# Franc-Z/CuClarabel

Measured on AMD Instinct MI355X. Metric: KKT factorize+solve/sec (fp64) per IPM iter, 100k-var SOCP, higher is better.
Workload: dtype f64

## Files before the change

cuclarabel_amd/csrc/factor_kernels.hip:

```cpp
#include "kernels.hpp"
#include "knobs.hpp"
#include <utility>

namespace hipkkt {

__device__ inline double rl_f64(double v, int lane)
{
    const int lo = __builtin_amdgcn_readlane(__double2loint(v), lane);
    const int hi = __builtin_amdgcn_readlane(__double2hiint(v), lane);
    return __hiloint2double(hi, lo);
}
#define WAVE_FENCE() asm volatile("" ::: "memory")

__device__ __forceinline__ void lds_add(double* p, double v)
{
    __hip_atomic_fetch_add(p, v, __ATOMIC_RELAXED, __HIP_MEMORY_SCOPE_WORKGROUP);
}
#define OV_LD(p) __hip_atomic_load((p), __ATOMIC_RELAXED, __HIP_MEMORY_SCOPE_AGENT)
#define OV_ST(p, v) __hip_atomic_store((p), (v), __ATOMIC_RELAXED, __HIP_MEMORY_SCOPE_AGENT)
__device__ inline bool ov_wait_ge(const int* counter, int target, int* abort_word, long long t0, long long limit, int who = 0, int info = 0,
                                  int* seen_min = nullptr)
{
    for (;;) {
        const int seen = __hip_atomic_load(counter, __ATOMIC_RELAXED, __HIP_MEMORY_SCOPE_AGENT);
// ... 4 lines not shown
            return false;
        }
        __builtin_amdgcn_s_sleep(2);
    }
}
__device__ inline int lower_bound_dev(const int* __restrict__ arr, int n, int v)
{
    int lo = 0, hi = n;
    while (lo < hi) {
        const int mid = (lo + hi) >> 1;
        if (arr[mid] < v) lo = mid + 1; else hi = mid;
    }
    return lo;
}

__global__ __launch_bounds__(256) void k_front_wave(FactorArgs A, int begin, int count, int slice)
{
    extern __shared__ __attribute__((aligned(16))) double smem[];
    const int lane = threadIdx.x & 63, wv = threadIdx.x >> 6;
    const int item = blockIdx.x * 4 + wv;
    if (item >= count) return;
    const TreeDev& T = A.T;
    const FrontDesc fd = T.desc[begin + item];
    const int s = fd.s, c0 = fd.c0, nc = fd.nc, nb = fd.nb;
    const int f = nc + nb;
    double* __restrict__ F = A.fronts + fd.front_off;
    double* __restrict__ U = A.upd + fd.upd_off;
    double* P = smem + (size_t)wv * slice;
    double* Us = P + f * nc;

    const bool pulled_leaf = (fd.pad & 2) != 0;
    for (int i = lane; i < f * nc + (pulled_leaf ? 0 : nb * nb); i += 64) P[i] = 0.0;
    WAVE_FENCE();
    {
        const int64_t e0 = fd.kptr;
        const int ne = fd.nk;
        for (int e = lane; e < ne; e += 64) P[T.kdst[e0 + e]] = A.Kval[T.ksrc[e0 + e]];
    }
    WAVE_FENCE();
    if (A.eps) {
        const double eps = *A.eps;
        if (lane < nc) P[lane + lane * f] += eps * (double)T.psign[c0 + lane];
    }
// ... 64 lines not shown
        WAVE_FENCE();
    }
    for (int i = lane; i < f * nc; i += 64) {
        const int j = i / f, r = i - j * f;
        if (r >= j) F[i] = P[i];
    }
    if (lane < nb && !pulled_leaf) {
        const int a = lane;
        for (int b = 0; b <= a; ++b) {
            double acc = 0.0;
            for (int k = 0; k < nc; ++k) acc = fma(P[nc + a + k * f] * P[k + k * f], P[nc + b + k * f], acc);
            U[a + (int64_t)b * nb] = Us[a + b * nb] - acc;
        }
    }
}

constexpr int kTinySlice = 128;
__global__ __launch_bounds__(256) void k_front_tiny(FactorArgs A, int begin, int count)
{
    __shared__ __attribute__((aligned(16))) double smem_t[32 * kTinySlice];
    const int sub = threadIdx.x & 7, grp = threadIdx.x >> 3;
    const int item = blockIdx.x * 32 + grp;
    if (item >= count) return;
    const TreeDev& T = A.T;
    const FrontDesc fd = T.desc[begin + item];
    const int s = fd.s, c0 = fd.c0, nc = fd.nc, nb = fd.nb;
    const int f = nc + nb;
    double* __restrict__ F = A.fronts + fd.front_off;
    double* __restrict__ U = A.upd + fd.upd_off;
    double* P = smem_t + grp * kTinySlice;
    double* Us = P + f * nc;

    const bool pulled_leaf = (fd.pad & 2) != 0;
    for (int i = sub; i < f * nc + (pulled_leaf ? 0 : nb * nb); i += 8) P[i] = 0.0;
    WAVE_FENCE();
    {
        const int64_t e0 = fd.kptr;
        const int ne = fd.nk;
        for (int e = sub; e < ne; e += 8) P[T.kdst[e0 + e]] = A.Kval[T.ksrc[e0 + e]];
    }
    WAVE_FENCE();
    if (A.eps) {
        const double eps = *A.eps;
        if (sub < nc) P[sub + sub * f] += eps * (double)T.psign[c0 + sub];
    }
// ... 38 lines not shown
        WAVE_FENCE();
    }
    for (int i = sub; i < f * nc; i += 8) {
        const int j = i / f, r = i - j * f;
        if (r >= j) F[i] = P[i];
    }
    if (sub < nb && !pulled_leaf) {
        const int a = sub;
        for (int b = 0; b <= a; ++b) {
            double acc = 0.0;
            for (int k = 0; k < nc; ++k) acc = fma(P[nc + a + k * f] * P[k + k * f], P[nc + b + k * f], acc);
            U[a + (int64_t)b * nb] = Us[a + b * nb] - acc;
        }
    }
}

typedef double d4_t __attribute__((ext_vector_type(4)));

__device__ inline double fast_recip(double d)
{
    double r = __builtin_amdgcn_rcp(d);
    r = fma(fma(-d, r, 1.0), r, r);
    r = fma(fma(-d, r, 1.0), r, r);
    return r;
}
constexpr int NB = kPanelNB;
__device__ __forceinline__ int pcol(int j, int f) { return (j * (2 * f - 1 - j)) >> 1; }

__device__ inline int64_t uniform_i64(int64_t v)
{
// ... 101 lines not shown
{
    int lo = __double2loint(v), hi = __double2hiint(v);
    switch (k) {
        HIPKKT_BCAST16_CASE(0) HIPKKT_BCAST16_CASE(1) HIPKKT_BCAST16_CASE(2) HIPKKT_BCAST16_CASE(3)
        HIPKKT_BCAST16_CASE(4) HIPKKT_BCAST16_CASE(5) HIPKKT_BCAST16_CASE(6) HIPKKT_BCAST16_CASE(7)
        HIPKKT_BCAST16_CASE(8) HIPKKT_BCAST16_CASE(9) HIPKKT_BCAST16_CASE(10) HIPKKT_BCAST16_CASE(11)
        HIPKKT_BCAST16_CASE(12) HIPKKT_BCAST16_CASE(13) HIPKKT_BCAST16_CASE(14) HIPKKT_BCAST16_CASE(15)
    }
    return __hiloint2double(hi, lo);
}

template <int BS, bool SLICED, bool OV>
__global__ __launch_bounds__(BS) void k_panel(FactorArgs A, int begin)
{
    extern __shared__ __attribute__((aligned(16))) double smem[];
    const int tid = threadIdx.x, lane = tid & 63;
    const int wv = __builtin_amdgcn_readfirstlane(tid >> 6);
    constexpr int NW = BS / 64;
    constexpr int NWK = NW - NW / 4;
    const int widx = wv - 1 - (wv >> 2);
    const TreeDev& T = A.T;
    const FrontDesc fd = SLICED ? T.sdesc[begin + blockIdx.x] : T.desc[begin + blockIdx.x];
    const int s = fd.s, c0 = fd.c0, nc = fd.nc, nb = fd.nb;
    const int ff = nc + nb;
    const int nsl = SLICED ? (fd.pad & 0xffff) : 1, sl = SLICED ? (fd.pad >> 16) : 0;
    const int rsmax = (nb + nsl - 1) / nsl;
    const int r_lo = nc + sl * rsmax;
    const int rs = SLICED ? max(0, min(rsmax, ff - r_lo)) : nb;
    const int f = nc + rs;
    const bool first = !SLICED || sl == 0;
    double* __restrict__ F = A.fronts + fd.front_off;
    if (OV && tid == 0) __hip_atomic_fetch_add(A.ov_started + A.ov_slot, 1, __ATOMIC_RELAXED, __HIP_MEMORY_SCOPE_AGENT);

    double* sh_d_all = smem;
    double* sh_dinv_all = smem + 2 * NB;
    double* Lb_all = smem + 4 * NB;
    double* colb = smem + 4 * NB + 2 * NB * NB;
    double* sgn = colb + 4 * NB;
    int* lds_cnt = reinterpret_cast<int*>(sgn + kBdCols + NB);
    double* P = sgn + kBdCols + NB + 2;

    HIPKKT_STAMP(A, 0);
    const long long clk0 = A.stamps ? clock64() : 0;
    const int64_t dense_off_s = T.dense_off[s];
    int64_t it0 = 0, it1 = 0;
    int pt0 = 0, pt1 = 0;
    PullGroup pt_first{};
    ExtItem it_first{};
    {
        const int64_t* __restrict__ wc = T.wave_cut + (int64_t)(SLICED ? T.nsuper + begin + (int)blockIdx.x : s) * 17;
        constexpr int SPW = 16 / NW > 0 ? 16 / NW : 1;
        if (wv * SPW < 16) {
            it0 = wc[wv * SPW];
            it1 = wc[min(16, (wv + 1) * SPW)];
            if (it1 > it0) it_first = T.items[min(it0 + lane, it1 - 1)];
            if (!SLICED) {
                pt0 = T.pwave_cut[(int64_t)s * 17 + wv * SPW];
                pt1 = T.pwave_cut[(int64_t)s * 17 + min(16, (wv + 1) * SPW)];
                pt0 = __builtin_amdgcn_readfirstlane(pt0);
                pt1 = __builtin_amdgcn_readfirstlane(pt1);
                if (pt1 > pt0) pt_first = pull_fetch(T.pterms, pt0, pt1, lane);
            }
        }
    }
    for (int k = tid; k < nc; k += BS) sgn[k] = (double)T.psign[c0 + k];
    const int psize = f * nc - ((nc * (nc - 1)) >> 1);
    for (int i = tid; i < psize; i += BS) P[i] = 0.0;
    __syncthreads();
    HIPKKT_STAMP(A, 1);
    {
        const int64_t e0 = fd.kptr;
        const int ne = fd.nk;
        for (int base = 0; base < ne; base += 4 * BS) {
            int src[4], dst[4];
            double v[4];
#pragma unroll
            for (int q = 0; q < 4; ++q) {
                const int e = base + q * BS + tid;
                src[q] = e < ne ? T.ksrc[e0 + e] : -1;
                dst[q] = e < ne ? T.kdst[e0 + e] : -1;
            }
#pragma unroll
            for (int q = 0; q < 4; ++q) v[q] = src[q] >= 0 ? A.Kval[src[q]] : 0.0;
#pragma unroll
            for (int q = 0; q < 4; ++q) if (dst[q] >= 0) P[dst[q]] = v[q];
        }
    }
    __syncthreads();
    if (A.eps) {
        const double eps = *A.eps;
        for (int k = tid; k < nc; k += BS) P[k + pcol(k, f)] += eps * sgn[k];
    }
    __syncthreads();
    HIPKKT_STAMP(A, 2);
    if (OV) {
        volatile int& sh_ov_ok = reinterpret_cast<volatile int*>(lds_cnt)[2];
        if (tid == 0) sh_ov_ok = 1;
        __syncthreads();
        if (wv == 0) {
            const long long tw = wall_clock64();
            bool ok = true;
            for (int e = T.child_ptr[s] + lane; e < T.child_ptr[s + 1]; e += 64) {
                const int c = T.child_idx[e];
                const int need = A.ov_ntiles[c];
                if (need > 0) ok = ov_wait_ge(A.ov_done + c, need, A.flags + 2, tw, A.ov_limit, 1, c) && ok;
            }
            if (!ok) sh_ov_ok = 0;
        }
        __syncthreads();
// ... 10 lines not shown
#pragma unroll
                for (int q = 0; q < 8; ++q) {
                    const int idx = base + q * BS + tid;
                    const int j = idx / f, rl = idx - j * f;
                    const int r = (!SLICED || rl < nc) ? rl : r_lo + (rl - nc);
                    const bool ok = idx < total && rl >= j;
                    tg[q] = ok ? rl + pcol(j, f) : -1;
                    v[q] = ok ? (OV ? OV_LD(Uc + r + (int64_t)j * ff) : Uc[r + (int64_t)j * ff]) : 0.0;
                }
#pragma unroll
                for (int q = 0; q < 8; ++q) if (tg[q] >= 0) P[tg[q]] += v[q];
            }
            __syncthreads();
        }
    }
    if (A.stamps && blockIdx.x == 0 && tid == 0) {
        asm volatile("s_waitcnt vmcnt(0)" ::: "memory");
        A.stamps[A.stamp_row * 16 + 6] = wall_clock64();
    }
    if (!SLICED && pt1 > pt0) apply_pulled(T.pterms, A.fronts, P, pt0, pt1, lane, pt_first);
    if (it1 > it0) apply_items_panel<SLICED, OV>(T, A.upd, P, f, it0, it1, lane, nc, r_lo, rs, it_first,
                                             (A.stamps && blockIdx.x == 0 && wv == 0) ? A.stamps + A.stamp_row * 16 + 15 : nullptr);
    if (A.stamps && blockIdx.x == 0 && tid == 0) A.stamps[A.stamp_row * 16 + 7] = wall_clock64();
    HIPKKT_STAMP(A, 3);
    long long t_i = 0, t_ii = 0, t_iii = 0, t0 = 0;
    auto diag_block = [&](const int kb, const int w, const int par) {
        double* sh_d = sh_d_all + par * NB;
        double* sh_dinv = sh_dinv_all + par * NB;
        double* Tb = Lb_all + par * NB * NB;
        int lane_o = lane;
        const int i = lane & 15, g = lane >> 4;
        const double my_sg = (lane < w) ? sgn[kb + lane] : 1.0;
        int nreg = 0;
        bool bad = false;
        double a4[4], lout[4], t4[4];
#pragma unroll
        for (int q = 0; q < 4; ++q) {
            const int j = 4 * g + q;
            a4[q] = (i < w && j <= i) ? P[(kb + i) + pcol(kb + j, f)] : 0.0;
// ... 129 lines not shown
                WAVE_FENCE();
                for (int idx = widx * 64 + lane; idx < w * f; idx += NWK * 64) {
                    const int jj = idx / f, r = idx - jj * f, j = kb + jj;
                    if (!SLICED) {
                        if (r >= j) OV_ST(F + r + (int64_t)j * ff, P[r + pcol(j, f)]);
                    } else if (r >= nc) {
                        OV_ST(F + (r_lo + r - nc) + (int64_t)j * ff, P[r + pcol(j, f)]);
                    } else if (first && r >= j) {
                        OV_ST(F + r + (int64_t)j * ff, P[r + pcol(j, f)]);
                    }
                }
                asm volatile("s_waitcnt vmcnt(0)" ::: "memory");
                if (lane == 0) {
                    const int arrived = __hip_atomic_fetch_add(lds_cnt + 1, 1, __ATOMIC_RELAXED, __HIP_MEMORY_SCOPE_WORKGROUP) + 1;
                    if (arrived == NWK * epoch)
                        __hip_atomic_store(SLICED ? A.ov_sprog + begin + blockIdx.x : A.ov_prog + s, kb + w, __ATOMIC_RELAXED,
                                           __HIP_MEMORY_SCOPE_AGENT);
                }
            }
            if (Tc > 0) {
                while (__hip_atomic_load(lds_cnt, __ATOMIC_RELAXED, __HIP_MEMORY_SCOPE_WORKGROUP) < (NWK + 1) * epoch)
                    __builtin_amdgcn_s_sleep(1);
                WAVE_FENCE();
                const int ntr = (Tr + 15) >> 4, ntc = (Tc + 15) >> 4;
                for (int t = widx; t < ntr * ntc; t += NWK) {
                    const int tc = t / ntr, tr = t - tc * ntr;
                    if (tr < tc || (tr == 0 && tc == 0)) continue;
                    tile(tr, tc);
                }
            }
        }
        if (A.stamps) { long long t1 = wall_clock64(); t_iii += t1 - t0; }
    }
    __syncthreads();
    HIPKKT_STAMP(A, 4);
    if (!OV) for (int idx = tid; idx < f * nc; idx += BS) {
        const int j = idx / f, r = idx - j * f;
        if (!SLICED) {
            if (r >= j) F[idx] = P[r + pcol(j, f)];
        } else if (r >= nc) {
            F[(r_lo + r - nc) + (int64_t)j * ff] = P[r + pcol(j, f)];
        } else if (first && r >= j) {
            F[r + (int64_t)j * ff] = P[r + pcol(j, f)];
        }
    }
    __syncthreads();
    HIPKKT_STAMP(A, 5);
    if (A.stamps && blockIdx.x == 0 && tid == 0) {
        A.stamps[A.stamp_row * 16 + 8] = t_i;
        A.stamps[A.stamp_row * 16 + 9] = t_ii;
        A.stamps[A.stamp_row * 16 + 10] = t_iii;
        A.stamps[A.stamp_row * 16 + 11] = f;
        A.stamps[A.stamp_row * 16 + 12] = nc;
        A.stamps[A.stamp_row * 16 + 13] = T.child_ptr[s + 1] - T.child_ptr[s];
        A.stamps[A.stamp_row * 16 + 14] = clock64() - clk0;
    }
}

constexpr int TS = 64;
constexpr int KC = 16;

constexpr int LDA = TS + 16;

// ... 230 lines not shown
static void init_factor_lds()
{
    static PerDeviceOnce once;
    once.run([]() {
        hipError_t e = hipSuccess;
        auto set = [&](auto k) { if (e == hipSuccess) e = set_max_lds(k, 160 * 1024); };
        set(k_panel<256, false, false>);
        set(k_panel<512, false, false>);
        set(k_panel<1024, false, false>);
        set(k_panel<256, false, true>);
        set(k_panel<512, false, true>);
        set(k_panel<1024, false, true>);
        set(k_panel<1024, true, false>);
        set(k_panel<1024, true, true>);
        set(k_front_wave);
        return e;
    });
}

void launch_front_tiny(const FactorArgs& a, int begin, int count, hipStream_t st)
{
    if (count <= 0) return;
    hipLaunchKernelGGL(k_front_tiny, dim3((count + 31) / 32), dim3(256), 0, st, a, begin, count);
}
void launch_front_wave(const FactorArgs& a, int begin, int count, int slice_doubles, hipStream_t st)
{
    if (count <= 0) return;
    init_factor_lds();
    hipLaunchKernelGGL(k_front_wave, dim3((count + 3) / 4), dim3(256), (size_t)4 * slice_doubles * sizeof(double), st,
                       a, begin, count, slice_doubles);
}
void launch_panel(const FactorArgs& a, int begin, int count, int bs, size_t lds, hipStream_t st)
{
    if (count <= 0) return;
    init_factor_lds();
    if (a.ov) {
        if (bs == 1024) hipLaunchKernelGGL((k_panel<1024, false, true>), dim3(count), dim3(1024), lds, st, a, begin);
        else if (bs == 512) hipLaunchKernelGGL((k_panel<512, false, true>), dim3(count), dim3(512), lds, st, a, begin);
        else hipLaunchKernelGGL((k_panel<256, false, true>), dim3(count), dim3(256), lds, st, a, begin);
        return;
    }
    if (bs == 1024) hipLaunchKernelGGL((k_panel<1024, false, false>), dim3(count), dim3(1024), lds, st, a, begin);
    else if (bs == 512) hipLaunchKernelGGL((k_panel<512, false, false>), dim3(count), dim3(512), lds, st, a, begin);
    else hipLaunchKernelGGL((k_panel<256, false, false>), dim3(count), dim3(256), lds, st, a, begin);
}
void launch_panel_sliced(const FactorArgs& a, int begin, int count, size_t lds, hipStream_t st)
{
    if (count <= 0) return;
    init_factor_lds();
    if (a.ov) hipLaunchKernelGGL((k_panel<1024, true, true>), dim3(count), dim3(1024), lds, st, a, begin);
    else hipLaunchKernelGGL((k_panel<1024, true, false>), dim3(count), dim3(1024), lds, st, a, begin);
}
void launch_schur(const FactorArgs& a, const int2* tiles, int tile_begin, int ntiles, hipStream_t st, int ov_grid, int tile_nc)
{
    if (ntiles <= 0) return;
    const int pipe_tiles = knobs().schur_pipe_tiles;
    const int pipe_nc = knobs().schur_pipe_nc;
    if (a.ov) hipLaunchKernelGGL((k_schur<true, true>), dim3(std::max(1, std::min(ntiles, ov_grid))), dim3(256), 0, st, a, tiles, tile_begin, ntiles);
    else if (ntiles > pipe_tiles && tile_nc >= pipe_nc) hipLaunchKernelGGL((k_schur<false, true>), dim3(ntiles), dim3(256), 0, st, a, tiles, tile_begin, ntiles);
// ... 65 lines not shown
```

cuclarabel_amd/csrc/hipkkt.hip:

```cpp
#include "../../include/hipkkt.h"

#include <hip/hip_runtime.h>

#include <algorithm>
#include <cfloat>
#include <chrono>
#include <climits>
#include <cmath>
#include <cstdio>
#include <cstdlib>
#include <cstring>
#include <array>
#include <functional>
#include <map>
#include <memory>
#include <mutex>
#include <stdexcept>
#include <string>
#include <vector>

#include "kernels.hpp"
#include "kkt_assembly.hpp"
#include "symbolic.hpp"
#include "knobs.hpp"
// ... 100 lines not shown
            }
            if (knobs().verbose >= 2)
                for (size_t q = 0; q < sch.launches.size(); ++q) {
                    const Launch& L = sch.launches[q];
                    int fmin = 1 << 30, ncmin = 1 << 30;
                    double flops = 0;
                    for (int t = L.begin; t < L.begin + L.count; ++t) {
                        const int sn = sch.sched[(size_t)t], nc = S.sn_start[sn + 1] - S.sn_start[sn], f = front_size(sn);
                        fmin = std::min(fmin, f); ncmin = std::min(ncmin, nc);
                        flops += (double)nc * (f - nc) * (f - nc) + (double)nc * nc * (f - nc) + (double)nc * nc * nc / 3;
                    }
                    std::fprintf(stderr, "[hipkkt] launch %zu level %d: %d fronts (%s), f %d..%d, nc %d..%d, %d sliced into %d, %d tiles (%d columns deep on average), %.3f GF\n",
                                 q, L.level, L.count, L.small ? "one wave" : "block", fmin, L.fmax, ncmin, L.ncmax, L.nsliced, L.slice_count,
                                 L.ntiles, L.tile_nc, flops * 1e-9);
                }
            if (overlap_wanted())
                for (size_t q = sch.ov_first; q < sch.launches.size(); ++q)
                    std::fprintf(stderr, "[hipkkt] overlap admission: launch %zu: %d panel workgroups, %d tiles behind a gate, %d CUs\n", q,
                                 sch.ov_group_of[q] >= 0 ? sch.ov_groups[(size_t)sch.ov_group_of[q]].count : sch.launches[q].count - sch.launches[q].nsliced + sch.launches[q].slice_count,
                                 sch.launches[q].ntiles, dev.n_cus);
        }
    }

    void factor(const double* d_Kval, const double* d_eps)
    {
        const bool want_stamps = knobs().stamps;
        const bool no_graph = !knobs().graph;
        if (want_stamps || no_graph || n_factor_calls++ == 0) {
            enqueue_factor(d_Kval, d_eps, stream, nullptr, want_stamps);
            return;
// ... 329 lines not shown
                    if (g->sliced) launch_panel_sliced(a, L.slice_begin, g->count, g->lds, st);
                    else launch_panel(a, L.begin, g->count, 1024, g->lds, st);
                }
                if (q == sch.ov_first) {
                    HIP_CHECK(hipEventRecord(ev_ov_fork, st));
                    HIP_CHECK(hipStreamWaitEvent(ov_stream, ev_ov_fork, 0));
                } else if (L.ntiles > 0 && !no_gate) {
                    if (merged) launch_ov_gate(d_ov_started.p + g->first, g->count, flags.p + 2, ov_limit, ov_stream);
                    else launch_ov_gate(d_ov_started.p + q, L.count - L.nsliced + L.slice_count, flags.p + 2, ov_limit, ov_stream);
                }
                launch_schur(a, (const int2*)d_tiles.p, L.tile_begin, L.ntiles, ov_stream, L.ntiles);
                a.ov = 0;
                continue;
            }
            if (L.small) {
                launch_front_wave(a, L.begin, L.count - L.ntiny, L.slice, st);
                launch_front_tiny(a, L.begin + L.count - L.ntiny, L.ntiny, st);
            } else {
                a.nbk = L.nbk;
                launch_panel(a, L.begin, L.count - L.nsliced, L.bs_panel, L.lds_panel, st);
                launch_panel_sliced(a, L.slice_begin, L.slice_count, L.lds_sliced, st);
                if (L.tinv_count > 0 && side) {
                    HIP_CHECK(hipEventRecord(ev_fork, st));
                    HIP_CHECK(hipStreamWaitEvent(side, ev_fork, 0));
                    form_w(d_tinv_list.p + L.tinv_begin, L.tinv_count, L.tinv_ncmax, side, 0);
                    forked = true;
                }
                launch_schur(a, (const int2*)d_tiles.p, L.tile_begin, L.ntiles, st, 0, L.tile_nc);
            }
        }
        if (forked) {
            HIP_CHECK(hipEventRecord(ev_join, side));
            HIP_CHECK(hipStreamWaitEvent(st, ev_join, 0));
        } else if (eager_fork) {
            const int done = w_done;
// ... 4091 lines not shown
```

cuclarabel_amd/csrc/kernels.hpp:

```cpp
#pragma once
#include <hip/hip_runtime.h>
#include "launch_shapes.hpp"
#include <cstdint>
#include <mutex>
#include <stdexcept>
#include <string>

namespace hipkkt {

struct HipError : std::runtime_error { using std::runtime_error::runtime_error; };

class PerDeviceOnce {
    std::mutex mu_;
    uint64_t done_[4] = {0, 0, 0, 0};
public:
    template <class F>
    void run(F&& fn)
    {
        int dev = 0;
        if (hipGetDevice(&dev) != hipSuccess || dev < 0 || dev >= 256) throw HipError("hipGetDevice failed");
        std::lock_guard<std::mutex> lk(mu_);
        if (done_[dev >> 6] >> (dev & 63) & 1) return;
        const hipError_t e = fn();
        if (e != hipSuccess) {
// ... 86 lines not shown
    double* fronts;
    double* upd;
    double* Dinv;
    int* flags;
    int* ov_prog;
    int* ov_done;
    const int* ov_ntiles;
    int* ov_sprog;
    const int* ov_sbase;
    int* ov_started;
    int ov_slot;
    int ov;
    long long ov_limit;
    double dyn_eps, dyn_delta;
    int nbk;
    long long* stamps;
    int stamp_row;
};
#define HIPKKT_STAMP(A, k) do { if ((A).stamps && blockIdx.x == 0 && threadIdx.x == 0) \
        (A).stamps[(A).stamp_row * 16 + (k)] = wall_clock64(); } while (0)

struct SolveArgs {
    TreeDev T;
    const double* fronts;
    const double* tinv;
    const double* Dinv;
    const double* b;
    double* out;
    double* xp;
    double* uvec;
    long long* top_stamps;
    long long top_limit;
    int64_t ld_b, ld_out, ld_xp, ld_uvec;
    const int* tk_pos;
// ... 7 lines not shown
};

constexpr int kSolveChunk = 128;
int top_solve_capacity(size_t lds, bool tall);
int top_solve_capacity_nr(size_t lds_total, int nr);
void launch_top_solve(const SolveArgs& a, int begin, int count, int grid, size_t lds, int* flags, int nflag, int epoch,
                      hipStream_t st, bool tall, int nr = 1);
int top_solve_sliced_capacity(size_t lds, int nr = 1);
void launch_top_solve_sliced(const SolveArgs& a, int begin, int pos0, int task0, int task1, int grid, size_t lds, int* flags, int nflag,
                             int epoch, hipStream_t st, int nr = 1);
void launch_tinv(const TreeDev& T, const double* fronts, double* tinv, const int* list, int count, int ncmax,
                 hipStream_t st, int max_blocks = 0, int nsmall = 0);

void launch_front_wave(const FactorArgs& a, int begin, int count, int slice_doubles, hipStream_t st);
void launch_front_tiny(const FactorArgs& a, int begin, int count, hipStream_t st);
void launch_panel(const FactorArgs& a, int begin, int count, int bs, size_t lds, hipStream_t st);
void launch_panel_sliced(const FactorArgs& a, int begin, int count, size_t lds, hipStream_t st);
void launch_schur(const FactorArgs& a, const int2* tiles, int tile_begin, int ntiles, hipStream_t st, int ov_grid = 0, int tile_nc = 0);
void launch_ov_gate(const int* started, int target, int* abort_word, long long limit, hipStream_t st);
void launch_concurrency_probe(int* word2, hipStream_t first, hipStream_t second);
void launch_handover_litmus(int variant, double* payload, int* sig, int* ack, int pairs, int words, int rounds,
                            unsigned long long* mismatches, unsigned long long* timeouts, hipStream_t st);
void launch_fwd(const SolveArgs& a, const RecSeg& rs, int begin, int count, int bs, size_t lds, hipStream_t st, int nr = 1);
void launch_bwd(const SolveArgs& a, const RecSeg& rs, int begin, int count, int bs, size_t lds, hipStream_t st, int nr = 1);
void launch_fwd_small(const SolveArgs& a, const RecSeg& rs, int begin, int nwave, int ntiny, hipStream_t st, bool leaf = false, int nr = 1);
void launch_bwd_small(const SolveArgs& a, const RecSeg& rs, int begin, int nwave, int ntiny, hipStream_t st, int nr = 1);
void launch_fwd_level(const SolveArgs& a, const RecSeg& rs, int begin, int nblock, int nwave, int ntiny, int bs, size_t lds, hipStream_t st, int nr = 1);
void launch_bwd_level(const SolveArgs& a, const RecSeg& rs, int begin, int nblock, int nwave, int ntiny, int bs, size_t lds, hipStream_t st, int nr = 1);

void launch_permute_in(const double* B, int64_t ldb, double* Xp, int KP, const int* iperm, int N, int nrhs, hipStream_t st);
// ... 299 lines not shown
```

cuclarabel_amd/csrc/knobs.hpp:

```cpp
#pragma once
#include <cstdlib>

namespace hipkkt {

#define HIPKKT_KNOBS(KNOB, FLAG_SET, FLAG_ON)                                                                                         \
                                                                                                                 \
    KNOB(int, verbose, "HIPKKT_VERBOSE", 0)                  \
    FLAG_SET(stamps, "HIPKKT_STAMPS")                                    \
    KNOB(int, top_stamps, "HIPKKT_TOP_STAMPS", 0)            \
    KNOB(int, top_stamps_nr, "HIPKKT_TOP_STAMPS_NR", 1)                                       \
    FLAG_SET(dump_levels, "HIPKKT_DUMP_LEVELS")                                \
    FLAG_SET(dump_subtrees, "HIPKKT_DUMP_SUBTREES")                        \
                                                                                      \
    KNOB(double, nd_sep_ratio, "HIPKKT_ND_SEP_RATIO", 0.10)  \
    KNOB(int, nd_sep_min, "HIPKKT_ND_SEP_MIN", 5000)                                           \
    KNOB(long long, panel_cap, "HIPKKT_PANEL_CAP", -1)       \
    KNOB(int, panel_max_cols, "HIPKKT_PANEL_MAX_COLS", -1)                                                  \
    KNOB(int, panel_slice_below, "HIPKKT_PANEL_SLICE_BELOW", -1)  \
    FLAG_SET(postorder_layout, "HIPKKT_POSTORDER_LAYOUT")                       \
    FLAG_ON(upd_pingpong, "HIPKKT_UPD_PINGPONG")                                        \
    KNOB(int, bundle_kids, "HIPKKT_BUNDLE_KIDS", 200)        \
    KNOB(int, bundle_kids_panel, "HIPKKT_BUNDLE_KIDS_PANEL", 400)   \
    FLAG_ON(bundle_cost, "HIPKKT_BUNDLE_COST")               \
                                                                                                  \
// ... 14 lines not shown
    FLAG_SET(graph, "HIPKKT_GRAPH")                               \
    FLAG_SET(no_overlap, "HIPKKT_NO_OVERLAP")                                                         \
    KNOB(int, winv_tail, "HIPKKT_WINV_TAIL", 4)                \
    KNOB(int, winv_early, "HIPKKT_WINV_EARLY", 1)                                                   \
    KNOB(int, winv_blocks, "HIPKKT_WINV_BLOCKS", 0)                           \
    FLAG_ON(winv_split, "HIPKKT_WINV_SPLIT")                 \
    FLAG_ON(winv_run_forks, "HIPKKT_WINV_RUN_FORKS")                        \
    FLAG_ON(factor_overlap, "HIPKKT_FACTOR_OVERLAP")                 \
    FLAG_SET(ov_cu_mask, "HIPKKT_OV_CU_MASK")                                        \
    KNOB(long long, ov_test_limit, "HIPKKT_OV_TEST_LIMIT", 5000000)   \
    KNOB(int, ov_max_fronts, "HIPKKT_OV_MAX_FRONTS", 0)      \
    KNOB(int, ov_max_tiles, "HIPKKT_OV_MAX_TILES", 1600)     \
    KNOB(int, ov_merge, "HIPKKT_OV_MERGE", 100)                   \
    KNOB(int, ov_merge_wide, "HIPKKT_OV_MERGE_WIDE", 24)                     \
    KNOB(int, ov_merge_groups, "HIPKKT_OV_MERGE_GROUPS", 8)                                \
    KNOB(int, schur_pipe_tiles, "HIPKKT_SCHUR_PIPE_TILES", 1600)                     \
    KNOB(int, schur_pipe_nc, "HIPKKT_SCHUR_PIPE_NC", 64)            \
                                                                                                                      \
    FLAG_SET(no_top, "HIPKKT_NO_TOP")                                                            \
    KNOB(int, top_tall, "HIPKKT_TOP_TALL", -1)                                        \
    KNOB(int, top_cap, "HIPKKT_TOP_CAP", 1 << 30)                                        \
    KNOB(double, top_mult, "HIPKKT_TOP_MULT", 1.5)                            \
    KNOB(long long, top_test_limit, "HIPKKT_TOP_TEST_LIMIT", 5000000)  \
    FLAG_SET(no_level_merge, "HIPKKT_NO_LEVEL_MERGE")               \
    KNOB(int, solve_slice_kb, "HIPKKT_SOLVE_SLICE_KB", 80)                                  \
    KNOB(int, solve_slice_max, "HIPKKT_SOLVE_SLICE_MAX", 64)                                     \
    KNOB(long long, solve_slice_from, "HIPKKT_SOLVE_SLICE_FROM", -1)  \
    FLAG_ON(chain, "HIPKKT_CHAIN")                                                           \
    FLAG_ON(chain_top, "HIPKKT_CHAIN_TOP")                   \
    KNOB(int, chain_max, "HIPKKT_CHAIN_MAX", 640)                                             \
// ... 35 lines not shown
```

cuclarabel_amd/csrc/launch_shapes.hpp:

```cpp
#pragma once
#include <cstddef>
#include <cstdint>

namespace hipkkt {

constexpr size_t kLdsCap = 160 * 1024 - 512;

constexpr int kLongRow = 4096;
constexpr int kLongChunk = 2048;

constexpr int kSmallFrontMax = 64;
constexpr int kSmallSliceMax = 1536;

constexpr int kPanelNB = 16;
constexpr int kMaxNbk = 16;
constexpr int kBdCols = 128;
inline size_t panel_lds_bytes(int fmax, int panel_max)
{
    (void)fmax;
    return ((size_t)8 * kPanelNB + 2 * kPanelNB * kPanelNB + (kBdCols + kPanelNB) + 2 + (size_t)panel_max + 256) * sizeof(double);
}

inline size_t solve_lds_bytes(int fmax, int ncmax)
{
    const size_t fpad = (size_t)((fmax + 3) & ~3), ncpad = (size_t)((ncmax + 3) & ~3);
    const size_t nks = (size_t)((ncmax + 7) >> 3), nrs = (size_t)((fmax + 7) >> 3);
    const size_t fwd = fpad + nks * fpad, bwd = fpad + nrs * ncpad;
// ... 60 lines not shown
```

cuclarabel_amd/csrc/schedule.cpp:

```cpp
#include "schedule.hpp"

#include <algorithm>
#include <cstdio>
#include <stdexcept>
#include <unordered_map>

namespace hipkkt {

static bool front_is_tall(const Symbolic& S, int s)
{
    const int tall_rows = knobs().solve_tall_rows;
    const int f = front_size(S, s), nc = S.sn_start[s + 1] - S.sn_start[s];
    return solve_lds_bytes(f, nc) > kLdsCap || (tall_rows > 0 && f >= tall_rows);
}

static void form_launches(const Symbolic& S, const DeviceLimits& dev, int64_t panel_cap, int panel_max_slices, Schedule& sch)
{
    sch.tile_base.assign(S.nsuper, -1);
    auto ncols = [&](int s) { return S.sn_start[s + 1] - S.sn_start[s]; };
    auto is_small = [&](int s) {
        int f = front_size(S, s), nc = ncols(s), nb = f - nc;
        return f <= kSmallFrontMax && f * nc + nb * nb <= kSmallSliceMax;
    };
    int level_no = -1;
// ... 276 lines not shown
        const int wgs = chain_seg_wgs(L.small ? 0 : L.count, L.small ? L.count - L.ntiny : 0, L.small ? L.ntiny : 0);
        if (L.ntall > 0 || (!L.small && L.lds_solve > 150 * 1024) || wgs > chain_max) break;
        if (!L.small) sch.chain_lds = std::max(sch.chain_lds, L.lds_solve);
        --q;
    }
    sch.chain_from = sch.launches.size() - q >= 2 ? q : sch.launches.size();
    sch.nch.assign((size_t)std::max(S.nsuper, 1), 0);
    if (sch.chain_from < sch.launches.size()) {
        const int p0 = sch.launches[sch.chain_from].begin;
        for (int c = 0; c < S.nsuper; ++c)
            if (S.sn_parent[c] >= 0 && sch.spos[(size_t)c] >= p0) sch.nch[(size_t)S.sn_parent[c]]++;
    }
}


Schedule build_schedule(const Symbolic& S, const DeviceLimits& dev, int64_t panel_cap, int panel_max_slices)
{
    Schedule sch;
    form_launches(S, dev, panel_cap, panel_max_slices, sch);
    admit_overlap(dev, sch);
    pick_late(sch);
    pick_top(S, dev, sch);
    pick_chain(S, sch);
    sch.rec_bytes = layout_records(sch.launches, &sch.rec_refused_bytes);
    return sch;
}

int rec_classes(const Launch& L, RecClass out[2])
{
    int n = 0;
    if (L.small) {
        if (L.count - L.ntiny > 0) out[n++] = {L.begin, L.count - L.ntiny, 1};
        if (L.ntiny > 0) out[n++] = {L.begin + L.count - L.ntiny, L.ntiny, 2};
    } else if (L.count > 0) {
        out[n++] = {L.begin, L.count, 0};
// ... 474 lines not shown
```

cuclarabel_amd/csrc/schedule.hpp:

```cpp
#pragma once
#include <array>
#include <cstddef>
#include <cstdint>
#include <functional>
#include <string>
#include <vector>

#include "knobs.hpp"
#include "launch_shapes.hpp"
#include "symbolic.hpp"

namespace hipkkt {

inline void apply_knobs(SymbolicOptions& opt)
{
    if (knobs().panel_cap >= 0) opt.panel_cap = knobs().panel_cap;
    if (knobs().panel_max_cols >= 0) opt.panel_max_cols = knobs().panel_max_cols;
    if (knobs().panel_slice_below >= 0) opt.panel_slice_below = knobs().panel_slice_below;
}

inline int front_size(const Symbolic& S, int s)
{
    return (S.sn_start[s + 1] - S.sn_start[s]) + (int)(S.rowptr[s + 1] - S.rowptr[s]);
}
// ... 10 lines not shown
    bool small;
    int bs_panel, nbk, slice;
    size_t lds_panel, lds_solve;
    int fmax, ncmax;
    int solve_bs;
    int ntiny;
    int tile_begin, ntiles;
    int tile_nc = 0;
    int tinv_begin, tinv_count, tinv_ncmax;
    int nsliced;
    int slice_begin, slice_count;
    size_t lds_sliced;
    int ntall;
    int level;
    RecSeg rec;
};

struct MergeGroup {
    size_t first, end;
    int count;
    size_t lds;
    bool sliced;
};

struct Schedule {
    std::vector<Launch> launches;
    std::vector<int> sched;
    std::vector<int> spos;
    std::vector<int64_t> tiles;
    std::vector<int64_t> tile_base;
// ... 78 lines not shown
inline bool pair_at(const Schedule& sch, size_t q, const SweepPlan& p)
{
    const std::vector<Launch>& launches = sch.launches;
    return p.merge_levels && q + 1 < p.nper && !launches[q].small && launches[q].ntall == 0 && launches[q + 1].small &&
           launches[q].level == launches[q + 1].level;
}
inline RecSeg pair_rec(const Launch& Lb, const Launch& Ls)
{
    RecSeg r = Ls.rec;
    r.off[0] = Lb.rec.off[0]; r.stride[0] = Lb.rec.stride[0]; r.fmax[0] = Lb.rec.fmax[0];
    return r;
}

std::string describe(const SweepPlan& p, const Schedule& sch, int nr, bool w_pending, bool packed);
std::string describe_launches(const SweepPlan& p, const Schedule& sch);

}
```

Before: 326.5.

## Fold small-front wave/tiny kernels into the panel launch as rider workgroups

Moves the small-front wave and tiny factorization work into extra workgroups of the preceding same-level panel kernel, or into a single combined small-front kernel when no panel launch is available. This removes one or two kernel launches per tree level and lets the small fronts run alongside the panel fronts. In exchange, the panel launch may need more LDS per workgroup, which can reduce occupancy. The tiny slice size also drops from 128 to 64 doubles.

```diff
diff --git a/cuclarabel_amd/csrc/factor_kernels.hip b/cuclarabel_amd/csrc/factor_kernels.hip
--- a/cuclarabel_amd/csrc/factor_kernels.hip
+++ b/cuclarabel_amd/csrc/factor_kernels.hip
@@ -42,19 +42,14 @@
     return lo;
 }
 
-__global__ __launch_bounds__(256) void k_front_wave(FactorArgs A, int begin, int count, int slice)
-{
-    extern __shared__ __attribute__((aligned(16))) double smem[];
-    const int lane = threadIdx.x & 63, wv = threadIdx.x >> 6;
-    const int item = blockIdx.x * 4 + wv;
-    if (item >= count) return;
+__device__ __forceinline__ void front_wave_body(const FactorArgs& A, double* P, int pos, int lane)
+{
     const TreeDev& T = A.T;
-    const FrontDesc fd = T.desc[begin + item];
+    const FrontDesc fd = T.desc[pos];
     const int s = fd.s, c0 = fd.c0, nc = fd.nc, nb = fd.nb;
     const int f = nc + nb;
     double* __restrict__ F = A.fronts + fd.front_off;
     double* __restrict__ U = A.upd + fd.upd_off;
-    double* P = smem + (size_t)wv * slice;
     double* Us = P + f * nc;
 
     const bool pulled_leaf = (fd.pad & 2) != 0;
@@ -149,21 +144,23 @@
         }
     }
 }
-
-constexpr int kTinySlice = 128;
-__global__ __launch_bounds__(256) void k_front_tiny(FactorArgs A, int begin, int count)
-{
-    __shared__ __attribute__((aligned(16))) double smem_t[32 * kTinySlice];
-    const int sub = threadIdx.x & 7, grp = threadIdx.x >> 3;
-    const int item = blockIdx.x * 32 + grp;
+__global__ __launch_bounds__(256) void k_front_wave(FactorArgs A, int begin, int count, int slice)
+{
+    extern __shared__ __attribute__((aligned(16))) double smem[];
+    const int lane = threadIdx.x & 63, wv = threadIdx.x >> 6;
+    const int item = blockIdx.x * 4 + wv;
     if (item >= count) return;
+    front_wave_body(A, smem + (size_t)wv * slice, begin + item, lane);
+}
+
+__device__ __forceinline__ void front_tiny_body(const FactorArgs& A, double* P, int pos, int sub)
+{
     const TreeDev& T = A.T;
-    const FrontDesc fd = T.desc[begin + item];
+    const FrontDesc fd = T.desc[pos];
     const int s = fd.s, c0 = fd.c0, nc = fd.nc, nb = fd.nb;
     const int f = nc + nb;
     double* __restrict__ F = A.fronts + fd.front_off;
     double* __restrict__ U = A.upd + fd.upd_off;
-    double* P = smem_t + grp * kTinySlice;
     double* Us = P + f * nc;
 
     const bool pulled_leaf = (fd.pad & 2) != 0;
@@ -232,6 +229,36 @@
         }
     }
 }
+__global__ __launch_bounds__(256) void k_front_tiny(FactorArgs A, int begin, int count)
+{
+    __shared__ __attribute__((aligned(16))) double smem_t[32 * kTinySlice];
+    const int sub = threadIdx.x & 7, grp = threadIdx.x >> 3;
+    const int item = blockIdx.x * 32 + grp;
+    if (item >= count) return;
+    front_tiny_body(A, smem_t + grp * kTinySlice, begin + item, sub);
+}
+
+__device__ __forceinline__ void small_riders(const FactorArgs& A, double* smem, int bx)
+{
+    const SmallRiders& R = A.rid;
+    const int nwb = R.wave_wgs();
+    if (bx < nwb) {
+        const int lane = threadIdx.x & 63, wv = threadIdx.x >> 6;
+        const int item = bx * R.fw + wv;
+        if (wv >= R.fw || item >= R.nwave) return;
+        front_wave_body(A, smem + (size_t)wv * R.slice, R.begin + item, lane);
+    } else {
+        const int sub = threadIdx.x & 7, grp = threadIdx.x >> 3;
+        const int item = (bx - nwb) * R.ft + grp;
+        if (grp >= R.ft || item >= R.ntiny) return;
+        front_tiny_body(A, smem + grp * kTinySlice, R.begin + R.nwave + item, sub);
+    }
+}
+__global__ __launch_bounds__(256) void k_front_small(FactorArgs A)
+{
+    extern __shared__ __attribute__((aligned(16))) double smem[];
+    small_riders(A, smem, blockIdx.x);
+}
 
 typedef double d4_t __attribute__((ext_vector_type(4)));
 
@@ -363,13 +390,19 @@
 __global__ __launch_bounds__(BS) void k_panel(FactorArgs A, int begin)
 {
     extern __shared__ __attribute__((aligned(16))) double smem[];
+    int bx = blockIdx.x;
+    if constexpr (!SLICED && !OV) {
+        const int nrid = A.rid.wgs();
+        if (bx < nrid) { small_riders(A, smem, bx); return; }
+        bx -= nrid;
+    }
     const int tid = threadIdx.x, lane = tid & 63;
     const int wv = __builtin_amdgcn_readfirstlane(tid >> 6);
     constexpr int NW = BS / 64;
     constexpr int NWK = NW - NW / 4;
     const int widx = wv - 1 - (wv >> 2);
     const TreeDev& T = A.T;
-    const FrontDesc fd = SLICED ? T.sdesc[begin + blockIdx.x] : T.desc[begin + blockIdx.x];
+    const FrontDesc fd = SLICED ? T.sdesc[begin + bx] : T.desc[begin + bx];
     const int s = fd.s, c0 = fd.c0, nc = fd.nc, nb = fd.nb;
     const int ff = nc + nb;
     const int nsl = SLICED ? (fd.pad & 0xffff) : 1, sl = SLICED ? (fd.pad >> 16) : 0;
@@ -389,7 +422,7 @@
     int* lds_cnt = reinterpret_cast<int*>(sgn + kBdCols + NB);
     double* P = sgn + kBdCols + NB + 2;
 
-    HIPKKT_STAMP(A, 0);
+    HIPKKT_STAMP(A, 0, bx);
     const long long clk0 = A.stamps ? clock64() : 0;
     const int64_t dense_off_s = T.dense_off[s];
     int64_t it0 = 0, it1 = 0;
@@ -397,7 +430,7 @@
     PullGroup pt_first{};
     ExtItem it_first{};
     {
-        const int64_t* __restrict__ wc = T.wave_cut + (int64_t)(SLICED ? T.nsuper + begin + (int)blockIdx.x : s) * 17;
+        const int64_t* __restrict__ wc = T.wave_cut + (int64_t)(SLICED ? T.nsuper + begin + bx : s) * 17;
         constexpr int SPW = 16 / NW > 0 ? 16 / NW : 1;
         if (wv * SPW < 16) {
             it0 = wc[wv * SPW];
@@ -416,7 +449,7 @@
     const int psize = f * nc - ((nc * (nc - 1)) >> 1);
     for (int i = tid; i < psize; i += BS) P[i] = 0.0;
     __syncthreads();
-    HIPKKT_STAMP(A, 1);
+    HIPKKT_STAMP(A, 1, bx);
     {
         const int64_t e0 = fd.kptr;
         const int ne = fd.nk;
@@ -441,7 +474,7 @@
         for (int k = tid; k < nc; k += BS) P[k + pcol(k, f)] += eps * sgn[k];
     }
     __syncthreads();
-    HIPKKT_STAMP(A, 2);
+    HIPKKT_STAMP(A, 2, bx);
     if (OV) {
         volatile int& sh_ov_ok = reinterpret_cast<volatile int*>(lds_cnt)[2];
         if (tid == 0) sh_ov_ok = 1;
@@ -482,15 +515,15 @@
             __syncthreads();
         }
     }
-    if (A.stamps && blockIdx.x == 0 && tid == 0) {
+    if (A.stamps && bx == 0 && tid == 0) {
         asm volatile("s_waitcnt vmcnt(0)" ::: "memory");
         A.stamps[A.stamp_row * 16 + 6] = wall_clock64();
     }
     if (!SLICED && pt1 > pt0) apply_pulled(T.pterms, A.fronts, P, pt0, pt1, lane, pt_first);
     if (it1 > it0) apply_items_panel<SLICED, OV>(T, A.upd, P, f, it0, it1, lane, nc, r_lo, rs, it_first,
-                                             (A.stamps && blockIdx.x == 0 && wv == 0) ? A.stamps + A.stamp_row * 16 + 15 : nullptr);
-    if (A.stamps && blockIdx.x == 0 && tid == 0) A.stamps[A.stamp_row * 16 + 7] = wall_clock64();
-    HIPKKT_STAMP(A, 3);
+                                             (A.stamps && bx == 0 && wv == 0) ? A.stamps + A.stamp_row * 16 + 15 : nullptr);
+    if (A.stamps && bx == 0 && tid == 0) A.stamps[A.stamp_row * 16 + 7] = wall_clock64();
+    HIPKKT_STAMP(A, 3, bx);
     long long t_i = 0, t_ii = 0, t_iii = 0, t0 = 0;
     auto diag_block = [&](const int kb, const int w, const int par) {
         double* sh_d = sh_d_all + par * NB;
@@ -650,7 +683,7 @@
                 if (lane == 0) {
                     const int arrived = __hip_atomic_fetch_add(lds_cnt + 1, 1, __ATOMIC_RELAXED, __HIP_MEMORY_SCOPE_WORKGROUP) + 1;
                     if (arrived == NWK * epoch)
-                        __hip_atomic_store(SLICED ? A.ov_sprog + begin + blockIdx.x : A.ov_prog + s, kb + w, __ATOMIC_RELAXED,
+                        __hip_atomic_store(SLICED ? A.ov_sprog + begin + bx : A.ov_prog + s, kb + w, __ATOMIC_RELAXED,
                                            __HIP_MEMORY_SCOPE_AGENT);
                 }
             }
@@ -669,7 +702,7 @@
         if (A.stamps) { long long t1 = wall_clock64(); t_iii += t1 - t0; }
     }
     __syncthreads();
-    HIPKKT_STAMP(A, 4);
+    HIPKKT_STAMP(A, 4, bx);
     if (!OV) for (int idx = tid; idx < f * nc; idx += BS) {
         const int j = idx / f, r = idx - j * f;
         if (!SLICED) {
@@ -681,8 +714,8 @@
         }
     }
     __syncthreads();
-    HIPKKT_STAMP(A, 5);
-    if (A.stamps && blockIdx.x == 0 && tid == 0) {
+    HIPKKT_STAMP(A, 5, bx);
+    if (A.stamps && bx == 0 && tid == 0) {
         A.stamps[A.stamp_row * 16 + 8] = t_i;
         A.stamps[A.stamp_row * 16 + 9] = t_ii;
         A.stamps[A.stamp_row * 16 + 10] = t_iii;
@@ -943,6 +976,7 @@
         set(k_panel<1024, true, false>);
         set(k_panel<1024, true, true>);
         set(k_front_wave);
+        set(k_front_small);
         return e;
     });
 }
@@ -958,6 +992,12 @@
     init_factor_lds();
     hipLaunchKernelGGL(k_front_wave, dim3((count + 3) / 4), dim3(256), (size_t)4 * slice_doubles * sizeof(double), st,
                        a, begin, count, slice_doubles);
+}
+void launch_front_small(const FactorArgs& a, size_t lds, hipStream_t st)
+{
+    if (a.rid.wgs() <= 0) return;
+    init_factor_lds();
+    hipLaunchKernelGGL(k_front_small, dim3(a.rid.wgs()), dim3(256), lds, st, a);
 }
 void launch_panel(const FactorArgs& a, int begin, int count, int bs, size_t lds, hipStream_t st)
 {
@@ -969,9 +1009,10 @@
         else hipLaunchKernelGGL((k_panel<256, false, true>), dim3(count), dim3(256), lds, st, a, begin);
         return;
     }
-    if (bs == 1024) hipLaunchKernelGGL((k_panel<1024, false, false>), dim3(count), dim3(1024), lds, st, a, begin);
-    else if (bs == 512) hipLaunchKernelGGL((k_panel<512, false, false>), dim3(count), dim3(512), lds, st, a, begin);
-    else hipLaunchKernelGGL((k_panel<256, false, false>), dim3(count), dim3(256), lds, st, a, begin);
+    const int grid = count + a.rid.wgs();
+    if (bs == 1024) hipLaunchKernelGGL((k_panel<1024, false, false>), dim3(grid), dim3(1024), lds, st, a, begin);
+    else if (bs == 512) hipLaunchKernelGGL((k_panel<512, false, false>), dim3(grid), dim3(512), lds, st, a, begin);
+    else hipLaunchKernelGGL((k_panel<256, false, false>), dim3(grid), dim3(256), lds, st, a, begin);
 }
 void launch_panel_sliced(const FactorArgs& a, int begin, int count, size_t lds, hipStream_t st)
 {
diff --git a/cuclarabel_amd/csrc/hipkkt.hip b/cuclarabel_amd/csrc/hipkkt.hip
--- a/cuclarabel_amd/csrc/hipkkt.hip
+++ b/cuclarabel_amd/csrc/hipkkt.hip
@@ -138,6 +138,7 @@
                                  q, L.level, L.count, L.small ? "one wave" : "block", fmin, L.fmax, ncmin, L.ncmax, L.nsliced, L.slice_count,
                                  L.ntiles, L.tile_nc, flops * 1e-9);
                 }
+            if (knobs().verbose >= 2) std::fputs(describe_factor_launches(sch, overlap_wanted()).c_str(), stderr);
             if (overlap_wanted())
                 for (size_t q = sch.ov_first; q < sch.launches.size(); ++q)
                     std::fprintf(stderr, "[hipkkt] overlap admission: launch %zu: %d panel workgroups, %d tiles behind a gate, %d CUs\n", q,
@@ -497,11 +498,20 @@
                 continue;
             }
             if (L.small) {
-                launch_front_wave(a, L.begin, L.count - L.ntiny, L.slice, st);
-                launch_front_tiny(a, L.begin + L.count - L.ntiny, L.ntiny, st);
+                if (L.rid_mode == 0) {
+                    launch_front_wave(a, L.begin, L.count - L.ntiny, L.slice, st);
+                    launch_front_tiny(a, L.begin + L.count - L.ntiny, L.ntiny, st);
+                } else if (L.rid_mode == 1) {
+                    a.rid = L.rid;
+                    launch_front_small(a, L.rid_lds, st);
+                    a.rid = SmallRiders{};
+                }
             } else {
                 a.nbk = L.nbk;
-                launch_panel(a, L.begin, L.count - L.nsliced, L.bs_panel, L.lds_panel, st);
+                const Launch* riders = q + 1 < nl && sch.launches[q + 1].small && sch.launches[q + 1].rid_mode == 2 ? &sch.launches[q + 1] : nullptr;
+                if (riders) a.rid = riders->rid;
+                launch_panel(a, L.begin, L.count - L.nsliced, L.bs_panel, riders ? riders->rid_lds : L.lds_panel, st);
+                a.rid = SmallRiders{};
                 launch_panel_sliced(a, L.slice_begin, L.slice_count, L.lds_sliced, st);
                 if (L.tinv_count > 0 && side) {
                     HIP_CHECK(hipEventRecord(ev_fork, st));
diff --git a/cuclarabel_amd/csrc/kernels.hpp b/cuclarabel_amd/csrc/kernels.hpp
--- a/cuclarabel_amd/csrc/kernels.hpp
+++ b/cuclarabel_amd/csrc/kernels.hpp
@@ -124,10 +124,11 @@
     long long ov_limit;
     double dyn_eps, dyn_delta;
     int nbk;
+    SmallRiders rid;
     long long* stamps;
     int stamp_row;
 };
-#define HIPKKT_STAMP(A, k) do { if ((A).stamps && blockIdx.x == 0 && threadIdx.x == 0) \
+#define HIPKKT_STAMP(A, k, bx) do { if ((A).stamps && (bx) == 0 && threadIdx.x == 0) \
         (A).stamps[(A).stamp_row * 16 + (k)] = wall_clock64(); } while (0)
 
 struct SolveArgs {
@@ -165,6 +166,7 @@
 
 void launch_front_wave(const FactorArgs& a, int begin, int count, int slice_doubles, hipStream_t st);
 void launch_front_tiny(const FactorArgs& a, int begin, int count, hipStream_t st);
+void launch_front_small(const FactorArgs& a, size_t lds, hipStream_t st);
 void launch_panel(const FactorArgs& a, int begin, int count, int bs, size_t lds, hipStream_t st);
 void launch_panel_sliced(const FactorArgs& a, int begin, int count, size_t lds, hipStream_t st);
 void launch_schur(const FactorArgs& a, const int2* tiles, int tile_begin, int ntiles, hipStream_t st, int ov_grid = 0, int tile_nc = 0);
diff --git a/cuclarabel_amd/csrc/knobs.hpp b/cuclarabel_amd/csrc/knobs.hpp
--- a/cuclarabel_amd/csrc/knobs.hpp
+++ b/cuclarabel_amd/csrc/knobs.hpp
@@ -52,6 +52,7 @@
     KNOB(int, ov_merge, "HIPKKT_OV_MERGE", 100)                   \
     KNOB(int, ov_merge_wide, "HIPKKT_OV_MERGE_WIDE", 24)                     \
     KNOB(int, ov_merge_groups, "HIPKKT_OV_MERGE_GROUPS", 8)                                \
+    KNOB(int, panel_riders, "HIPKKT_PANEL_RIDERS", 1)        \
     KNOB(int, schur_pipe_tiles, "HIPKKT_SCHUR_PIPE_TILES", 1600)                     \
     KNOB(int, schur_pipe_nc, "HIPKKT_SCHUR_PIPE_NC", 64)            \
                                                                                                                       \
diff --git a/cuclarabel_amd/csrc/launch_shapes.hpp b/cuclarabel_amd/csrc/launch_shapes.hpp
--- a/cuclarabel_amd/csrc/launch_shapes.hpp
+++ b/cuclarabel_amd/csrc/launch_shapes.hpp
@@ -1,6 +1,13 @@
 #pragma once
+#include <algorithm>
 #include <cstddef>
 #include <cstdint>
+
+#if defined(__HIPCC__)
+#define HIPKKT_HD __host__ __device__
+#else
+#define HIPKKT_HD
+#endif
 
 namespace hipkkt {
 
@@ -11,6 +18,21 @@
 
 constexpr int kSmallFrontMax = 64;
 constexpr int kSmallSliceMax = 1536;
+
+constexpr int kTinySlice = 64;
+struct SmallRiders {
+    int begin = 0;
+    int nwave = 0, ntiny = 0;
+    int slice = 0;
+    int fw = 1, ft = 1;
+    int nwb = 0, ntb = 0;
+    void fit(int fw_, int ft_) { fw = fw_ > 1 ? fw_ : 1; ft = ft_ > 1 ? ft_ : 1; nwb = (nwave + fw - 1) / fw; ntb = (ntiny + ft - 1) / ft; }
+    HIPKKT_HD int wave_wgs() const { return nwb; }
+    HIPKKT_HD int tiny_wgs() const { return ntb; }
+    HIPKKT_HD int wgs() const { return nwb + ntb; }
+};
+inline int riders_fw(int threads, size_t lds, int slice) { return slice > 0 ? (int)std::min<size_t>((size_t)threads / 64, lds / ((size_t)slice * sizeof(double))) : threads / 64; }
+inline int riders_ft(int threads, size_t lds) { return (int)std::min<size_t>((size_t)threads / 8, lds / (kTinySlice * sizeof(double))); }
 
 constexpr int kPanelNB = 16;
 constexpr int kMaxNbk = 16;
diff --git a/cuclarabel_amd/csrc/schedule.cpp b/cuclarabel_amd/csrc/schedule.cpp
--- a/cuclarabel_amd/csrc/schedule.cpp
+++ b/cuclarabel_amd/csrc/schedule.cpp
@@ -314,11 +314,74 @@
 }
 
 
+static void plan_riders(Schedule& sch)
+{
+    const int knob = knobs().panel_riders;
+    constexpr size_t kTinyBytes = kTinySlice * sizeof(double);
+    for (size_t q = 0; q < sch.launches.size(); ++q) {
+        Launch& L = sch.launches[q];
+        L.rid_mode = 0;
+        L.rid = SmallRiders{};
+        L.rid_lds = 0;
+        if (!L.small || knob <= 0) continue;
+        SmallRiders R;
+        R.begin = L.begin;
+        R.nwave = L.count - L.ntiny;
+        R.ntiny = L.ntiny;
+        R.slice = L.slice;
+        const size_t wave_b = R.nwave > 0 ? (size_t)L.slice * sizeof(double) : 0, tiny_b = R.ntiny > 0 ? kTinyBytes : 0;
+        if (q > 0) {
+            const Launch& B = sch.launches[q - 1];
+            if (!B.small && B.level == L.level && B.count - B.nsliced > 0) {
+                size_t best = 0;
+                for (int k = 1; k <= B.bs_panel / 64; ++k) {
+                    const size_t lds = std::max({B.lds_panel, (size_t)k * wave_b, tiny_b});
+                    if (lds > kLdsCap) continue;
+                    SmallRiders C = R;
+                    C.fit(riders_fw(B.bs_panel, lds, R.slice), riders_ft(B.bs_panel, lds));
+                    const size_t total = (size_t)(B.count - B.nsliced + C.wgs()) * lds;
+                    if (L.rid_mode != 2 || total < best) { best = total; L.rid_mode = 2; L.rid = C; L.rid_lds = lds; }
+                    if (R.nwave == 0) break;
+                }
+                if (L.rid_mode == 2) continue;
+            }
+        }
+        if (R.nwave > 0 && R.ntiny > 0) {
+            int k = 1;
+            while (k < 4 && (size_t)k * wave_b < 32 * kTinyBytes) ++k;
+            const size_t lds = std::max((size_t)k * wave_b, 32 * kTinyBytes);
+            R.fit(riders_fw(256, lds, R.slice), riders_ft(256, lds));
+            L.rid_mode = 1; L.rid = R; L.rid_lds = lds;
+        }
+    }
+}
+
+std::string describe_factor_launches(const Schedule& sch, bool overlap)
+{
+    std::string out;
+    char buf[320];
+    for (size_t q = 0; q < sch.launches.size(); ++q) {
+        const Launch& L = sch.launches[q];
+        if (L.small) {
+            std::snprintf(buf, sizeof buf, "[hipkkt] factor launch %zu level %d: family %s wave %d tiny %d fw %d ft %d lds %zu\n", q, L.level,
+                          L.rid_mode == 2 ? "rides" : (L.rid_mode == 1 ? "small" : "wave+tiny"), L.count - L.ntiny, L.ntiny, L.rid.fw, L.rid.ft, L.rid_lds);
+        } else {
+            const Launch* R = q + 1 < sch.launches.size() && sch.launches[q + 1].small && sch.launches[q + 1].rid_mode == 2 ? &sch.launches[q + 1] : nullptr;
+            std::snprintf(buf, sizeof buf, "[hipkkt] factor launch %zu level %d: family panel bs %d whole %d sliced %d overlapped %d riders wave %d tiny %d workgroups %d lds %zu\n",
+                          q, L.level, L.bs_panel, L.count - L.nsliced, L.slice_count, overlap && q >= sch.ov_first ? 1 : 0, R ? R->rid.nwave : 0, R ? R->rid.ntiny : 0,
+                          R ? R->rid.wgs() : 0, R ? R->rid_lds : L.lds_panel);
+        }
+        out += buf;
+    }
+    return out;
+}
+
 Schedule build_schedule(const Symbolic& S, const DeviceLimits& dev, int64_t panel_cap, int panel_max_slices)
 {
     Schedule sch;
     form_launches(S, dev, panel_cap, panel_max_slices, sch);
     admit_overlap(dev, sch);
+    plan_riders(sch);
     pick_late(sch);
     pick_top(S, dev, sch);
     pick_chain(S, sch);
diff --git a/cuclarabel_amd/csrc/schedule.hpp b/cuclarabel_amd/csrc/schedule.hpp
--- a/cuclarabel_amd/csrc/schedule.hpp
+++ b/cuclarabel_amd/csrc/schedule.hpp
@@ -48,6 +48,9 @@
     int ntall;
     int level;
     RecSeg rec;
+    int rid_mode = 0;
+    SmallRiders rid;
+    size_t rid_lds = 0;
 };
 
 struct MergeGroup {
@@ -156,5 +159,6 @@
 
 std::string describe(const SweepPlan& p, const Schedule& sch, int nr, bool w_pending, bool packed);
 std::string describe_launches(const SweepPlan& p, const Schedule& sch);
+std::string describe_factor_launches(const Schedule& sch, bool overlap = true);
 
 }
```

Result: faster. 330.5 (median of 6 runs) (+1.2%).
